# wsntxxn/TextToAudioGrounding

Hardware: AMD Instinct MI355X
Metric: clips/sec (10 s@32 kHz, 1-phrase) fwd+bwd (higher is better)
Workload: dtype f32

## Files before the change

### texttoaudiogrounding_amd/csrc/conv_c1.hip

```cpp
#include "tag_common.h"

namespace {

__device__ __forceinline__ float c1_in(const float* x, const float* cs, const float* ct, int H, int W, long m,
                                       int h, int w, int dy, int dx) {
    const int hh = h + dy, ww = w + dx;
    if (hh < 0 || hh >= H || ww < 0 || ww >= W) return 0.0f;
    const float v = x[m + (long)dy * W + dx];
    return cs ? fmaf(v, cs[ww], ct[ww]) : v;
}

__global__ __launch_bounds__(256) void conv_c1_fwd_kernel(const float* __restrict__ x, const float* __restrict__ cs,
                                                          const float* __restrict__ ct, const float* __restrict__ w,
                                                          float* __restrict__ y, long M, int H, int W, int Cout) {
    const int C4 = Cout >> 2;
    const long total = M * C4;
    for (long i = (long)blockIdx.x * 256 + threadIdx.x; i < total; i += (long)gridDim.x * 256) {
        const int c = (int)(i % C4) << 2;
        const long m = i / C4;
        const int hw = (int)(m % ((long)H * W));
        const int h = hw / W, ww = hw % W;
        float o[4] = {0, 0, 0, 0};
#pragma unroll
        for (int tap = 0; tap < 9; ++tap) {
// ... 194 lines not shown
}

constexpr int C1B_GW = 66, C1B_GT = 10;
__device__ __forceinline__ void c1_stage_row(float (*Xs)[C1B_GW], const float* ximg, const float* cs, const float* ct, int H,
                                             int row) {
    constexpr int W = 64;
    const int tid = threadIdx.x;
    if (tid < C1B_GW) {
        const int w = tid - 1;
        float v = 0.0f;
        if ((unsigned)row < (unsigned)H && (unsigned)w < (unsigned)W) {
            v = ximg[(size_t)row * W + w];
            if (cs) v = fmaf(v, cs[w], ct[w]);
        }
        Xs[(row + 8) & 3][tid] = v;
    }
}

template <class TS>
__global__ __launch_bounds__(256) void conv_c1_fwd_rows_kernel(const float* __restrict__ x, const float* __restrict__ cs,
                                                               const float* __restrict__ ct, const float* __restrict__ wgt,
                                                               TS* __restrict__ y, float* __restrict__ stats, int H,
                                                               int strips, int rows_per_strip) {
    constexpr int W = 64, Cout = 64;
    __shared__ float Xs[4][C1B_GW];
    const int img = blockIdx.x / strips, strip = blockIdx.x % strips;
    const int r0 = strip * rows_per_strip;
    int r1 = r0 + rows_per_strip;
    if (r1 > H) r1 = H;
    const int tid = threadIdx.x, c = (tid & 15) << 2, grp = tid >> 4;
    float wr[4][9];
#pragma unroll
    for (int j = 0; j < 4; ++j)
#pragma unroll
        for (int t = 0; t < 9; ++t) wr[j][t] = wgt[(c + j) * 9 + t];
    const float* ximg = x + (size_t)img * H * W;
    float sk[4] = {0, 0, 0, 0}, sr[4] = {0, 0, 0, 0}, sq[4] = {0, 0, 0, 0};
    bool have_pivot = false;
    c1_stage_row(Xs, ximg, cs, ct, H, r0 - 1);
    c1_stage_row(Xs, ximg, cs, ct, H, r0);
    c1_stage_row(Xs, ximg, cs, ct, H, r0 + 1);
    __syncthreads();
    for (int h = r0; h < r1; ++h) {
        if (h + 2 <= r1) c1_stage_row(Xs, ximg, cs, ct, H, h + 2);
        float xin[3][6];
#pragma unroll
        for (int r = 0; r < 3; ++r)
#pragma unroll
            for (int k = 0; k < 6; ++k) xin[r][k] = Xs[(h + r - 1 + 8) & 3][grp * 4 + k];
        TS* yrow = y + (((size_t)img * H + h) * W + grp * 4) * Cout + c;
#pragma unroll
        for (int px = 0; px < 4; ++px) {
            float o[4] = {0, 0, 0, 0};
#pragma unroll
            for (int tap = 0; tap < 9; ++tap)
#pragma unroll
                for (int j = 0; j < 4; ++j) o[j] = fmaf(xin[tap / 3][px + tap % 3], wr[j][tap], o[j]);
            Act<TS>::st4(yrow + (size_t)px * Cout, (f32x4){o[0], o[1], o[2], o[3]});
            if (stats) {
                if (!have_pivot) {
#pragma unroll
                    for (int j = 0; j < 4; ++j) sk[j] = o[j];
                    have_pivot = true;
                }
#pragma unroll
                for (int j = 0; j < 4; ++j) { const float d = o[j] - sk[j]; sr[j] += d; sq[j] = fmaf(d, d, sq[j]); }
            }
        }
        __syncthreads();
    }
    if (stats) {
        const int P = gridDim.x * 16, prow = blockIdx.x * 16 + grp;
        float* ps = stats + (size_t)prow * 3 * Cout;
#pragma unroll
        for (int j = 0; j < 4; ++j) { ps[c + j] = sk[j]; ps[Cout + c + j] = sr[j]; ps[2 * Cout + c + j] = sq[j]; }
        if (c == 0) stats[(size_t)P * 3 * Cout + prow] = (float)((r1 - r0) * 4);
    }
}

struct C1BnBwd {
    const void* yref; const float* scale; const float* shift; const float* mean; const float* invstd;
    const float* gamma; const float* dgamma; const float* dbeta; float invN; int bn_train;
};
template <class TS, bool FUSE>
__global__ __launch_bounds__(256) void conv_c1_bwd_kernel(const float* __restrict__ x, const float* __restrict__ cs,
                                                          const float* __restrict__ ct, const TS* __restrict__ dy,
                                                          const float* __restrict__ wgt, float* __restrict__ dx,
                                                          double* __restrict__ partials, int H, int strips,
                                                          int rows_per_strip, C1BnBwd bb) {
    constexpr int W = 64, Cout = 64;
    __shared__ float Gs[4][C1B_GW][C1B_GT];
    __shared__ float Xs[4][C1B_GW];
    __shared__ float red[4][16][36];
    const int img = blockIdx.x / strips, strip = blockIdx.x % strips;
    const int r0 = strip * rows_per_strip;
    int r1 = r0 + rows_per_strip;
    if (r1 > H) r1 = H;
    const int tid = threadIdx.x, lane = tid & 63, wid = tid >> 6;
    const int cq = lane & 15, c = cq << 2, psub = lane >> 4;
    const int tapl = lane & 15, kg = lane >> 4;
    const bool tap_ok = tapl < 9;
    const int tky = tap_ok ? tapl / 3 : 0, tkx = tap_ok ? tapl % 3 : 0;
    float wB[16];
#pragma unroll
    for (int q = 0; q < 16; ++q) wB[q] = tap_ok ? wgt[(kg * 16 + q) * 9 + tapl] : 0.0f;
    f32x4 accW[4];
#pragma unroll
    for (int j = 0; j < 4; ++j) accW[j] = (f32x4){0.0f, 0.0f, 0.0f, 0.0f};
    __shared__ __attribute__((aligned(16))) float Ts[4][16][68];
    for (int i = tid; i < 4 * C1B_GW * C1B_GT; i += 256) (&Gs[0][0][0])[i] = 0.0f;
    const float* ximg = x + (size_t)img * H * W;
    const TS* dimg = dy + (size_t)img * H * W * Cout;
    typedef ActN<TS, 4> AN;
    typedef typename AN::raw_t raw_t;
    constexpr int NY = FUSE ? 4 : 1;
    f32x4 g[4];
    raw_t gn[4], yn[NY];
    __shared__ float bnc[7][Cout];
    const TS* yimg = nullptr;
    if constexpr (FUSE) {
        yimg = static_cast<const TS*>(bb.yref) + (size_t)img * H * W * Cout;
        if (tid < Cout) {
            const float is = bb.invstd[tid];
            bnc[0][tid] = bb.scale[tid]; bnc[1][tid] = bb.shift[tid]; bnc[2][tid] = bb.mean[tid]; bnc[3][tid] = is;
            bnc[4][tid] = bb.gamma[tid] * is;
            bnc[5][tid] = bb.bn_train ? bb.dbeta[tid] * bb.invN : 0.0f;
            bnc[6][tid] = bb.bn_train ? bb.dgamma[tid] * bb.invN : 0.0f;
        }
    }
    auto load_dy = [&](int row) {
        const bool ok = (unsigned)row < (unsigned)H;
        const size_t off = ((size_t)(ok ? row : 0) * W + wid * 16 + psub) * Cout + c;
#pragma unroll
        for (int i = 0; i < 4; ++i) {
            gn[i] = AN::ldraw(dimg + off + (size_t)i * 4 * Cout);
            if constexpr (FUSE) yn[i] = AN::ldraw(yimg + off + (size_t)i * 4 * Cout);
            else if (!ok) gn[i] = AN::zero();
        }
    };
    auto take = [&](bool ok) {
        if constexpr (FUSE) {
            float k[7][4];
#pragma unroll
            for (int q = 0; q < 7; ++q) {
                const f32x4 v = *reinterpret_cast<const f32x4*>(&bnc[q][c]);
                k[q][0] = v.x; k[q][1] = v.y; k[q][2] = v.z; k[q][3] = v.w;
            }
#pragma unroll
            for (int i = 0; i < 4; ++i) {
                float av[4], vv[4], o[4];
                AN::unpack(gn[i], av);
                AN::unpack(yn[i], vv);
#pragma unroll
                for (int j = 0; j < 4; ++j) {
                    const float dz = fmaf(vv[j], k[0][j], k[1][j]) > 0.0f ? av[j] : 0.0f;
                    o[j] = k[4][j] * (dz - k[5][j] - (vv[j] - k[2][j]) * k[3][j] * k[6][j]);
                    if (!ok) o[j] = 0.0f;
                }
                g[i] = (f32x4){o[0], o[1], o[2], o[3]};
            }
        } else {
#pragma unroll
            for (int i = 0; i < 4; ++i) {
                float av[4];
                AN::unpack(gn[i], av);
                g[i] = (f32x4){av[0], av[1], av[2], av[3]};
            }
        }
    };
    c1_stage_row(Xs, ximg, cs, ct, H, r0 - 1);
    c1_stage_row(Xs, ximg, cs, ct, H, r0);
    load_dy(r0 - 1);
    __syncthreads();
    take((unsigned)(r0 - 1) < (unsigned)H);
    for (int h = r0 - 1; h <= r1; ++h) {
        c1_stage_row(Xs, ximg, cs, ct, H, h + 2 > r1 + 1 ? -1 : h + 2);
        if (h < r1) load_dy(h + 1);
        const bool own = h >= r0 && h < r1;
        const int gs = (h + 8) & 3;
        if (own) {
#pragma unroll
            for (int i = 0; i < 4; ++i) {
                const float xb = tap_ok ? Xs[(h + tky - 1 + 8) & 3][wid * 16 + i * 4 + psub + tkx] : 0.0f;
                accW[0] = __builtin_amdgcn_mfma_f32_16x16x4f32(g[i].x, xb, accW[0], 0, 0, 0);
                accW[1] = __builtin_amdgcn_mfma_f32_16x16x4f32(g[i].y, xb, accW[1], 0, 0, 0);
                accW[2] = __builtin_amdgcn_mfma_f32_16x16x4f32(g[i].z, xb, accW[2], 0, 0, 0);
                accW[3] = __builtin_amdgcn_mfma_f32_16x16x4f32(g[i].w, xb, accW[3], 0, 0, 0);
            }
        }
#pragma unroll
        for (int i = 0; i < 4; ++i) *reinterpret_cast<f32x4*>(&Ts[wid][i * 4 + psub][c]) = g[i];
        __builtin_amdgcn_fence(__ATOMIC_RELEASE, "wavefront");
        __builtin_amdgcn_wave_barrier();
        __builtin_amdgcn_fence(__ATOMIC_ACQUIRE, "wavefront");
        f32x4 accG = (f32x4){0.0f, 0.0f, 0.0f, 0.0f};
#pragma unroll
        for (int q4 = 0; q4 < 4; ++q4) {
            const f32x4 v = *reinterpret_cast<const f32x4*>(&Ts[wid][tapl][kg * 16 + 4 * q4]);
            accG = __builtin_amdgcn_mfma_f32_16x16x4f32(v.x, wB[4 * q4 + 0], accG, 0, 0, 0);
            accG = __builtin_amdgcn_mfma_f32_16x16x4f32(v.y, wB[4 * q4 + 1], accG, 0, 0, 0);
            accG = __builtin_amdgcn_mfma_f32_16x16x4f32(v.z, wB[4 * q4 + 2], accG, 0, 0, 0);
            accG = __builtin_amdgcn_mfma_f32_16x16x4f32(v.w, wB[4 * q4 + 3], accG, 0, 0, 0);
        }
        if (tap_ok) {
            float* gp = &Gs[gs][wid * 16 + 4 * kg + 1][tapl];
            gp[0] = accG.x; gp[C1B_GT] = accG.y; gp[2 * C1B_GT] = accG.z; gp[3 * C1B_GT] = accG.w;
        }
        __syncthreads();
        const int ho = h - 1;
        if (ho >= r0 && ho < r1 && tid < W) {
            float sdx = 0.0f;
#pragma unroll
            for (int t = 0; t < 9; ++t)
                sdx += Gs[(ho - (t / 3 - 1) + 8) & 3][tid + 1 - (t % 3 - 1)][t];
            dx[((size_t)img * H + ho) * W + tid] = sdx;
        }
        if (h < r1) take((unsigned)(h + 1) < (unsigned)H);
    }
    if (tap_ok) {
#pragma unroll
        for (int j = 0; j < 4; ++j) {
            red[wid][4 * kg + 0][j * 9 + tapl] = accW[j].x;
            red[wid][4 * kg + 1][j * 9 + tapl] = accW[j].y;
            red[wid][4 * kg + 2][j * 9 + tapl] = accW[j].z;
            red[wid][4 * kg + 3][j * 9 + tapl] = accW[j].w;
        }
    }
    __syncthreads();
    for (int e = tid; e < 16 * 36; e += 256) {
        const int q = e / 36, r = e % 36;
        const double sum = ((double)red[0][q][r] + (double)red[1][q][r]) + ((double)red[2][q][r] + (double)red[3][q][r]);
        partials[(size_t)blockIdx.x * Cout * 9 + (q * 4 + r / 9) * 9 + r % 9] = sum;
    }
}

}

static void c1_bwd_geom(int B, int H, int* strips, int* rows) {
    int s = 2048 / (B > 0 ? B : 1);
    if (s < 1) s = 1;
    int r = (H + s - 1) / s;
    if (r < 8) r = 8;
    *rows = r;
    *strips = (H + r - 1) / r;
}
static int c1_blocks(long items, long per_block) {
    const long nb = (items + per_block - 1) / per_block;
    return (int)(nb > 8192 ? 8192 : nb);
}
template <class TS>
static int c1_fwd_rows_launch(const float* x, const float* col_scale, const float* col_shift, const float* w, TS* y,
                              float* stats, int B, int H, void* stream) {
    int strips, rows;
    c1_bwd_geom(B, H, &strips, &rows);
    hipLaunchKernelGGL(conv_c1_fwd_rows_kernel<TS>, dim3(B * strips), dim3(256), 0, as_stream(stream), x, col_scale, col_shift, w,
                       y, stats, H, strips, rows);
    TAG_LAUNCH_CHECK();
    return 0;
}

extern "C" int tag_conv3x3_c1_forward(const float* x, const float* col_scale, const float* col_shift, const float* w,
                                      float* y, int B, int H, int W, int Cout, void* stream) {
    TAG_CHECK_ARG(x && w && y && B > 0 && H > 0 && W > 0 && Cout > 0);
    TAG_CHECK_ARG(Cout % 4 == 0 && (col_scale == nullptr) == (col_shift == nullptr));
    const long M = (long)B * H * W;
    if (W == 64 && Cout == 64) return c1_fwd_rows_launch<float>(x, col_scale, col_shift, w, y, nullptr, B, H, stream);
    if (W % 4 == 0 && 256 % (Cout / 4) == 0)
        hipLaunchKernelGGL(conv_c1_fwd4_kernel<false>, dim3(c1_blocks((M / 4) * (Cout / 4), 256)), dim3(256), 0,
                           as_stream(stream), x, col_scale, col_shift, w, (const float*)nullptr, y, M, H, W, Cout);
    else
        hipLaunchKernelGGL(conv_c1_fwd_kernel, dim3(c1_blocks(M * (Cout / 4), 256)), dim3(256), 0, as_stream(stream), x,
                           col_scale, col_shift, w, y, M, H, W, Cout);
    TAG_LAUNCH_CHECK();
    return 0;
}

extern "C" int tag_conv3x3_c1_forward_bias(const float* x, const float* col_scale, const float* col_shift, const float* w,
                                           const float* bias, float* y, int B, int H, int W, int Cout, void* stream) {
    TAG_CHECK_ARG(x && w && bias && y && B > 0 && H > 0 && (col_scale == nullptr) == (col_shift == nullptr));
    if (!(W > 0 && W % 4 == 0 && Cout >= 4 && Cout % 4 == 0 && 256 % (Cout / 4) == 0)) {
        tag_set_error("%s", "tag_conv3x3_c1_forward_bias: unserved shape (W a multiple of 4, Cout / 4 a divisor of 256)");
        return TAG_EINVAL;
    }
    const long M = (long)B * H * W;
    hipLaunchKernelGGL(conv_c1_fwd4_kernel<true>, dim3(c1_blocks((M / 4) * (Cout / 4), 256)), dim3(256), 0, as_stream(stream), x,
                       col_scale, col_shift, w, bias, y, M, H, W, Cout);
    TAG_LAUNCH_CHECK();
    return 0;
}

extern "C" int tag_conv3x3_c1_stats_rows(int B, int H, int W, int Cout) {
    if (!(W == 64 && Cout == 64 && B > 0 && H > 0)) return 0;
    int strips, rows;
    c1_bwd_geom(B, H, &strips, &rows);
    return B * strips * 16;
}
extern "C" int tag_conv3x3_c1_forward_stats(const float* x, const float* col_scale, const float* col_shift, const float* w,
                                            float* y, float* stats, int B, int H, int W, int Cout, void* stream) {
    TAG_CHECK_ARG(x && w && y && stats && W == 64 && Cout == 64 && B > 0 && H > 0);
    TAG_CHECK_ARG((col_scale == nullptr) == (col_shift == nullptr));
    return c1_fwd_rows_launch<float>(x, col_scale, col_shift, w, y, stats, B, H, stream);
}
extern "C" int tag_conv3x3_c1_forward_stats_bf16(const float* x, const float* col_scale, const float* col_shift,
                                                 const float* w, void* y, float* stats, int B, int H, int W, int Cout,
                                                 void* stream) {
    TAG_CHECK_ARG(x && w && y && W == 64 && Cout == 64 && B > 0 && H > 0);
    TAG_CHECK_ARG((col_scale == nullptr) == (col_shift == nullptr));
    return c1_fwd_rows_launch<bf16_t>(x, col_scale, col_shift, w, static_cast<bf16_t*>(y), stats, B, H, stream);
}

extern "C" size_t tag_conv3x3_c1_wgrad_ws_bytes(int B, int H, int W, int Cout) {
    (void)B; (void)H; (void)W;
    return (size_t)1024 * Cout * 9 * sizeof(double);
}

extern "C" int tag_conv3x3_c1_wgrad(const float* x, const float* col_scale, const float* col_shift, const float* dy,
                                    float* dw, int B, int H, int W, int Cout, void* ws, void* stream) {
    TAG_CHECK_ARG(x && dy && dw && ws && B > 0 && H > 0 && W > 0 && Cout > 0);
    TAG_CHECK_ARG(Cout % 4 == 0 && Cout / 4 <= 64 && 64 % (Cout / 4) == 0);
    TAG_CHECK_ARG((col_scale == nullptr) == (col_shift == nullptr));
    const long M = (long)B * H * W;
    const int rpi = 256 / (Cout / 4);
    long nb = (M + (long)rpi * 64 - 1) / ((long)rpi * 64);
    const int nblk = (int)(nb > 1024 ? 1024 : (nb < 1 ? 1 : nb));
    double* partials = static_cast<double*>(ws);
    hipLaunchKernelGGL(W % 4 == 0 ? conv_c1_wgrad_kernel<4> : conv_c1_wgrad_kernel<1>, dim3(nblk), dim3(256),
                       4 * 64 * 36 * sizeof(double), as_stream(stream), x, col_scale, col_shift, dy, partials, M, H, W, Cout);
    TAG_LAUNCH_CHECK();
    hipLaunchKernelGGL(conv_c1_wgrad_finalize_kernel, dim3(cdiv(Cout * 9, 8)), dim3(256), 0, as_stream(stream),
                       partials, nblk, Cout * 9, dw);
    TAG_LAUNCH_CHECK();
    return 0;
}

extern "C" int tag_conv3x3_c1_dgrad(const float* dy, const float* w, float* dx, int B, int H, int W, int Cout,
                                    void* stream) {
    TAG_CHECK_ARG(dy && w && dx && B > 0 && H > 0 && W > 0 && Cout > 0);
    TAG_CHECK_ARG(Cout % 4 == 0 && Cout / 4 <= 64 && 64 % (Cout / 4) == 0);
    const long M = (long)B * H * W;
    const int rpi = 256 / (Cout / 4);
    hipLaunchKernelGGL(conv_c1_dgrad_kernel, dim3(c1_blocks(M, rpi)), dim3(256), 0, as_stream(stream), dy, w, dx, M, H, W, Cout);
    TAG_LAUNCH_CHECK();
    return 0;
}

extern "C" size_t tag_conv3x3_c1_backward_ws_bytes(int B, int H, int W, int Cout) {
    (void)W;
    int strips, rows;
    c1_bwd_geom(B, H, &strips, &rows);
    return (size_t)B * strips * Cout * 9 * sizeof(double);
}
template <class TS>
static int c1_backward_impl(const float* x, const float* col_scale, const float* col_shift, const TS* dy, const float* w,
                            float* dw, float* dx, int B, int H, int W, int Cout, void* ws, void* stream, const C1BnBwd* bb) {
    TAG_CHECK_ARG(x && dy && w && dw && dx && ws && B > 0 && H > 0);
    TAG_CHECK_ARG(W == 64 && Cout == 64);
    TAG_CHECK_ARG((col_scale == nullptr) == (col_shift == nullptr));
    int strips, rows;
    c1_bwd_geom(B, H, &strips, &rows);
    double* partials = static_cast<double*>(ws);
    if (bb) {
        TAG_CHECK_ARG(bb->yref && bb->scale && bb->shift && bb->mean && bb->invstd && bb->gamma && bb->dgamma && bb->dbeta);
        hipLaunchKernelGGL((conv_c1_bwd_kernel<TS, true>), dim3(B * strips), dim3(256), 0, as_stream(stream), x, col_scale,
                           col_shift, dy, w, dx, partials, H, strips, rows, *bb);
    } else {
        hipLaunchKernelGGL((conv_c1_bwd_kernel<TS, false>), dim3(B * strips), dim3(256), 0, as_stream(stream), x, col_scale,
                           col_shift, dy, w, dx, partials, H, strips, rows, C1BnBwd{});
    }
    TAG_LAUNCH_CHECK();
    hipLaunchKernelGGL(conv_c1_wgrad_finalize_kernel, dim3(cdiv(Cout * 9, 8)), dim3(256), 0, as_stream(stream),
                       partials, B * strips, Cout * 9, dw);
    TAG_LAUNCH_CHECK();
    return 0;
}
extern "C" int tag_conv3x3_c1_backward(const float* x, const float* col_scale, const float* col_shift, const float* dy,
                                       const float* w, float* dw, float* dx, int B, int H, int W, int Cout, void* ws,
                                       void* stream) {
    return c1_backward_impl<float>(x, col_scale, col_shift, dy, w, dw, dx, B, H, W, Cout, ws, stream, nullptr);
}
extern "C" int tag_conv3x3_c1_backward_bf16(const float* x, const float* col_scale, const float* col_shift, const void* dy,
                                            const float* w, float* dw, float* dx, int B, int H, int W, int Cout, void* ws,
                                            void* stream) {
    return c1_backward_impl<bf16_t>(x, col_scale, col_shift, static_cast<const bf16_t*>(dy), w, dw, dx, B, H, W, Cout, ws,
                                    stream, nullptr);
}
static C1BnBwd c1_bn_bwd(const void* yref, const float* bn_scale, const float* bn_shift, const float* bn_mean,
                         const float* bn_invstd, const float* gamma, const float* dgamma, const float* dbeta, int bn_train,
                         int B, int H, int W) {
    return C1BnBwd{yref, bn_scale, bn_shift, bn_mean, bn_invstd, gamma, dgamma, dbeta, 1.0f / (float)((long)B * H * W), bn_train};
}
extern "C" int tag_conv3x3_c1_backward_bnrelu(const float* x, const float* col_scale, const float* col_shift, const float* da,
                                              const float* yref, const float* bn_scale, const float* bn_shift,
                                              const float* bn_mean, const float* bn_invstd, const float* gamma,
                                              const float* dgamma, const float* dbeta, int bn_train, const float* w,
                                              float* dw, float* dx, int B, int H, int W, int Cout, void* ws, void* stream) {
    const C1BnBwd bb = c1_bn_bwd(yref, bn_scale, bn_shift, bn_mean, bn_invstd, gamma, dgamma, dbeta, bn_train, B, H, W);
    return c1_backward_impl<float>(x, col_scale, col_shift, da, w, dw, dx, B, H, W, Cout, ws, stream, &bb);
}
extern "C" int tag_conv3x3_c1_backward_bnrelu_bf16(const float* x, const float* col_scale, const float* col_shift,
                                                   const void* da, const void* yref, const float* bn_scale,
                                                   const float* bn_shift, const float* bn_mean, const float* bn_invstd,
                                                   const float* gamma, const float* dgamma, const float* dbeta, int bn_train,
                                                   const float* w, float* dw, float* dx, int B, int H, int W, int Cout,
                                                   void* ws, void* stream) {
    const C1BnBwd bb = c1_bn_bwd(yref, bn_scale, bn_shift, bn_mean, bn_invstd, gamma, dgamma, dbeta, bn_train, B, H, W);
    return c1_backward_impl<bf16_t>(x, col_scale, col_shift, static_cast<const bf16_t*>(da), w, dw, dx, B, H, W, Cout, ws,
                                    stream, &bb);
}
```

### texttoaudiogrounding_amd/csrc/tag_lib.hip

```cpp
#include <stdarg.h>
#include <string.h>
#include "tag_common.h"

static thread_local char g_err[512] = "";

void tag_set_error(const char* fmt, ...) {
    va_list ap;
    va_start(ap, fmt);
    vsnprintf(g_err, sizeof(g_err), fmt, ap);
    va_end(ap);
}

#ifndef TAG_CSRC_SHA256
#define TAG_CSRC_SHA256 "unknown"
#endif
namespace {
struct TagOpt { const char* name; int value; };
TagOpt g_opts[] = {
    {"conv_impl", 0},
    {"halo_lds_pad", 0},
    {"halo_bn256", 1},
    {"wgrad_wgs", 512},
    {"conv_rows", 1},
    {"wgrad_dma", 1},
    {"x3_products", 6},
    {"gemm_big_min", 2048},
    {"gru_tile4", 1},
    {"gru_xcd", 1},
    {"gru_coop", 1},
    {"mha_mfma", 1},
};
}
int tag_option(const char* name) {
    for (const TagOpt& o : g_opts)
        if (strcmp(o.name, name) == 0) return o.value;
    return 0;
}
extern "C" int tag_set_option(const char* name, int value) {
    TAG_CHECK_ARG(name != nullptr);
    for (TagOpt& o : g_opts)
        if (strcmp(o.name, name) == 0) { o.value = value; return 0; }
    tag_set_error("tag_set_option: unknown option '%s'", name);
    return TAG_EINVAL;
}

extern "C" int tag_abi_version(void) { return TAG_ABI_VERSION; }
extern "C" const char* tag_build_id(void) { return TAG_CSRC_SHA256; }
extern "C" const char* tag_last_error(void) { return g_err; }
extern "C" int tag_device_cu_count(void) {
    int dev = 0, n = 0;
    if (hipGetDevice(&dev) != hipSuccess) return -1;
    if (hipDeviceGetAttribute(&n, hipDeviceAttributeMultiprocessorCount, dev) != hipSuccess) return -1;
    return n;
}

extern "C" int tag_stream_create_cu_mask(const unsigned* mask, int words, void** stream_out) {
    TAG_CHECK_ARG(mask && words > 0 && stream_out);
    hipStream_t st = nullptr;
    const hipError_t e = hipExtStreamCreateWithCUMask(&st, (uint32_t)words, mask);
    if (e != hipSuccess) {
        tag_set_error("hipExtStreamCreateWithCUMask failed: %s", hipGetErrorString(e));
        (void)hipGetLastError();
        return (int)e;
    }
    *stream_out = reinterpret_cast<void*>(st);
    return 0;
}
```

### texttoaudiogrounding_amd/dispatch.py

```python
from __future__ import annotations

import collections
import math
from typing import Optional

import torch

from . import settings as cfg
from .lib import call, ptr, query
from .engine import (F32, _chk, _empty, _timed, _ws)


def waveform_f16_to_f32_padded(clips, device, length=None):
    import numpy as np
    arrs = [c.numpy() if isinstance(c, torch.Tensor) else np.asarray(c) for c in clips]
    if any(a.dtype != np.float16 or a.ndim != 1 for a in arrs):
        raise RuntimeError("waveform_f16_to_f32_padded: clips must be 1-D float16 arrays (the pack's storage type)")
    lens = [a.shape[0] for a in arrs]
    S = int(length) if length is not None else max(lens)
    off = torch.tensor([0] + list(np.cumsum(lens)), dtype=torch.long)
    packed = torch.from_numpy(np.concatenate(arrs) if len(arrs) > 1 else arrs[0].copy())
    dev = torch.device(device)
    if dev.type != "cuda":
        raise RuntimeError("waveform_f16_to_f32_padded: the target must be the MI355X (cuda) device; no CPU fallback")
# ... 318 lines not shown
            ws = _ws(query("tag_conv3x3_wino_ws_bytes", b1 - b0, H, W, Cin, Cout), x)
            with _timed(("conv3x3_wino", b1 - b0, H, W, Cin, Cout), _wino_flop(b1 - b0, H, W, Cin, Cout)):
                call("tag_conv3x3_wino_forward_bnrelu_pool_eval", ptr(x[b0:b1]), ptr(u), prologue, ptr(scale), ptr(shift),
                     ptr(out[b0:b1]), ptr(st.scale), ptr(st.shift), b1 - b0, H, W, Cin, Cout, ph, pw, int(pool), ptr(ws))
        return out
    with _timed(("conv3x3_halo_kernel", B, H, W, Cin, Cout), 2.0 * B * H * W * 9 * Cin * Cout):
        call("tag_conv3x3_forward_bnrelu_pool_eval", ptr(x), ptr(wpack), prologue, ptr(scale), ptr(shift), ptr(out), ptr(st.scale),
             ptr(st.shift), B, H, W, Cin, Cout, ph, pw, int(pool))
    return out


def conv3x3_wgrad(x, dy, prologue=0, scale=None, shift=None, out=None):
    B, H, W, Cin = x.shape
    Cout = dy.shape[3]
    dw = out if out is not None else _empty(Cout, Cin, 3, 3, like=x)
    if x.dtype == BF16:
        if dy.dtype != BF16 or not (W in (8, 16, 32, 64) and Cin % 64 == 0 and Cout % 64 == 0):
            raise RuntimeError("bf16 wgrad: both operands must be bf16, width 8/16/32/64, channels multiples of 64")
        ws = _ws(query("tag_conv3x3_wgrad_x3_ws_bytes", B, H, W, Cin, Cout), x)
        with _timed(("conv3x3_wgrad_x3_kernel", B, H, W, Cin, Cout), 2.0 * B * H * W * 9 * Cin * Cout):
            call("tag_conv3x3_wgrad_x3_bf16", ptr(x), prologue, ptr(scale), ptr(shift), ptr(dy), ptr(dw), B, H, W, Cin, Cout,
                 ptr(ws))
        return dw
    if cfg.CONV_MATH in _X3_PRODUCTS and W in (8, 16, 32, 64) and Cin % 64 == 0 and Cout % 64 == 0:
        ws = _ws(query("tag_conv3x3_wgrad_x3_ws_bytes", B, H, W, Cin, Cout), x)
        with _timed(("conv3x3_wgrad_x3_kernel", B, H, W, Cin, Cout), 2.0 * B * H * W * 9 * Cin * Cout):
            call("tag_conv3x3_wgrad_x3", ptr(x), prologue, ptr(scale), ptr(shift), ptr(dy), ptr(dw), B, H, W, Cin, Cout,
                 _X3_PRODUCTS[cfg.CONV_MATH], ptr(ws))
        return dw
    if (x.dtype == F32 and dy.dtype == F32 and _wino_shape(W, Cin, Cout)
            and B * ((H + 1) // 2) * ((W + 1) // 2) * max(Cin, Cout) >= cfg.WINO_MIN_WORK and query("tag_conv3x3_wino_ok", B, H, W, Cin, Cout)):
        cfg.WINO_LAUNCHES += 1
        ws = _ws(query("tag_conv3x3_wino_wgrad_ws_bytes", B, H, W, Cin, Cout), x)
        with _timed(("conv3x3_wino_wgrad", B, H, W, Cin, Cout), _wino_flop(B, H, W, Cin, Cout)):
            call("tag_conv3x3_wino_wgrad", ptr(x), prologue, ptr(scale), ptr(shift), ptr(dy), ptr(dw), B, H, W, Cin, Cout, ptr(ws),
                 None)
        return dw
    ws = _ws(query("tag_conv3x3_wgrad_ws_bytes", B, H, W, Cin, Cout), x)
    kname = "conv3x3_wgrad_alltaps_kernel" if W in (8, 16, 32, 64) else "conv3x3_wgrad_kernel"
    with _timed((kname, B, H, W, Cin, Cout), 2.0 * B * H * W * 9 * Cin * Cout):
        call("tag_conv3x3_wgrad", ptr(x), prologue, ptr(scale), ptr(shift), ptr(dy), ptr(dw), B, H, W, Cin, Cout,
             ptr(ws))
    return dw


def conv3x3_c1(x, w, col_scale=None, col_shift=None):
    return conv3x3_c1_stats(x, w, col_scale, col_shift, want_stats=False)[0]


def conv3x3_c1_stats(x, w, col_scale=None, col_shift=None, want_stats=True, out_dtype=F32):
    B, H, W = x.shape
    Cout = w.shape[0]
    y = _empty(B, H, W, Cout, like=x, dtype=out_dtype)
    if out_dtype == BF16:
        P = query("tag_conv3x3_c1_stats_rows", B, H, W, Cout)
        if P <= 0:
            raise RuntimeError("bf16 activations: the Cin = 1 convolution is implemented for 64 mel bins x 64 channels")
        part = (P, _empty(P * (3 * Cout + 1), like=x)) if want_stats else None
        call("tag_conv3x3_c1_forward_stats_bf16", ptr(x), ptr(col_scale), ptr(col_shift), ptr(w), ptr(y),
             ptr(part[1]) if part else None, B, H, W, Cout)
        return y, part
    P = query("tag_conv3x3_c1_stats_rows", B, H, W, Cout) if (want_stats and cfg.FUSE_BN_STATS) else 0
    if P > 0:
        part = (P, _empty(P * (3 * Cout + 1), like=x))
        call("tag_conv3x3_c1_forward_stats", ptr(x), ptr(col_scale), ptr(col_shift), ptr(w), ptr(y), ptr(part[1]), B, H, W,
             Cout)
        return y, part
    call("tag_conv3x3_c1_forward", ptr(x), ptr(col_scale), ptr(col_shift), ptr(w), ptr(y), B, H, W, Cout)
    return y, None


def conv3x3_c1_wgrad(x, dy, col_scale=None, col_shift=None, out=None):
    B, H, W = x.shape
    Cout = dy.shape[3]
    dw = out if out is not None else _empty(Cout, 1, 3, 3, like=x)
    ws = _ws(query("tag_conv3x3_c1_wgrad_ws_bytes", B, H, W, Cout), x)
    call("tag_conv3x3_c1_wgrad", ptr(x), ptr(col_scale), ptr(col_shift), ptr(dy), ptr(dw), B, H, W, Cout, ptr(ws))
    return dw


C1_BWD_FUSED_SHAPE = (64, 64)


def conv3x3_c1_backward(x, dy, w, col_scale=None, col_shift=None, out=None, bn_bwd=None):
    B, H, W = x.shape
    Cout = dy.shape[3]
    if (W, Cout) == C1_BWD_FUSED_SHAPE:
        dw = out if out is not None else _empty(Cout, 1, 3, 3, like=x)
        dx = _empty(B, H, W, like=x)
        ws = _ws(query("tag_conv3x3_c1_backward_ws_bytes", B, H, W, Cout), x)
        if bn_bwd is not None:
            yref, st, gamma, dg, db = bn_bwd
            if yref.dtype != dy.dtype or yref.shape != dy.shape:
                raise RuntimeError("conv3x3_c1_backward: yref and da must agree in dtype and shape")
            call("tag_conv3x3_c1_backward_bnrelu" + _sfx(dy), ptr(x), ptr(col_scale), ptr(col_shift), ptr(dy), ptr(yref),
                 ptr(st.scale), ptr(st.shift), ptr(st.mean), ptr(st.invstd), ptr(gamma), ptr(dg), ptr(db), int(st.train),
                 ptr(w), ptr(dw), ptr(dx), B, H, W, Cout, ptr(ws))
            return dw, dx
        call("tag_conv3x3_c1_backward" + _sfx(dy), ptr(x), ptr(col_scale), ptr(col_shift), ptr(dy), ptr(w), ptr(dw), ptr(dx),
             B, H, W, Cout, ptr(ws))
        return dw, dx
    if bn_bwd is not None:
        raise RuntimeError("conv3x3_c1_backward: bn_bwd needs the fused 64 x 64 shape")
    if dy.dtype == BF16:
        raise RuntimeError("bf16 activations: the Cin = 1 backward is implemented for 64 mel bins x 64 channels")
    return conv3x3_c1_wgrad(x, dy, col_scale, col_shift), conv3x3_c1_dgrad(dy, w)


def conv3x3_c1_dgrad(dy, w):
    B, H, W, Cout = dy.shape
    dx = _empty(B, H, W, like=dy)
    call("tag_conv3x3_c1_dgrad", ptr(dy), ptr(w), ptr(dx), B, H, W, Cout)
    return dx


def bnact_pool(y, st: Optional[BNStat], ph, pw, act=1, pool=0, drop_p=0.0, seed=0):
    B, H, W, C = y.shape
    out = _empty(B, H // ph, W // pw, C, like=y, dtype=y.dtype)
    call("tag_bnact_pool_forward" + _sfx(y), ptr(y), ptr(st.scale) if st else None, ptr(st.shift) if st else None, ptr(out), B,
         H, W, C, ph, pw, act, pool, float(drop_p), seed)
    return out


def bnrelu_pool_backward(y, st: BNStat, gamma, dout, ph, pw, drop_p=0.0, seed=0, dg_out=None, db_out=None, pool=0,
                         partials=None):
    B, H, W, C = y.shape
    if dout.dtype != y.dtype:
        raise RuntimeError("bnrelu_pool_backward: y and dout must share their storage type")
    dy = _empty(B, H, W, C, like=y, dtype=y.dtype)
    dg, db = _dg_db(dg_out, db_out, C, y)
    if partials is not None:
        P, part = partials
        ws = _ws(query("tag_bn_grad_from_partials_ws_bytes", P, C), y)
        call("tag_bn_grad_from_partials", ptr(part), P, C, ptr(dg), ptr(db), ptr(ws))
        call("tag_bnrelu_pool_backward_apply" + _sfx(y), ptr(y), ptr(st.scale), ptr(st.shift), ptr(st.mean), ptr(st.invstd),
             ptr(gamma), ptr(dout), ptr(dy), ptr(dg), ptr(db), B, H, W, C, ph, pw, int(pool), float(drop_p), seed, int(st.train))
        return dy, dg, db
    ws = _ws(query("tag_bn_backward_ws_bytes", B * H * W, C), y)
    call("tag_bnrelu_pool_backward" + _sfx(y), ptr(y), ptr(st.scale), ptr(st.shift), ptr(st.mean), ptr(st.invstd), ptr(gamma),
         ptr(dout), ptr(dy), ptr(dg), ptr(db), B, H, W, C, ph, pw, int(pool), float(drop_p), seed, int(st.train), ptr(ws))
    return dy, dg, db


def bnrelu_backward(y, st: BNStat, gamma, da, inplace=True, dg_out=None, db_out=None):
    C = y.shape[-1]
    rows = y.numel() // C
    dy = da if inplace else torch.empty_like(da)
    dg, db = _dg_db(dg_out, db_out, C, y)
    ws = _ws(query("tag_bn_backward_ws_bytes", rows, C), y)
    if da.dtype != y.dtype:
        raise RuntimeError("bnrelu_backward: y and da must share their storage type")
    call("tag_bnrelu_backward" + _sfx(y), ptr(y), ptr(st.scale), ptr(st.shift), ptr(st.mean), ptr(st.invstd), ptr(gamma),
         ptr(da), ptr(dy), ptr(dg), ptr(db), rows, C, int(st.train), ptr(ws))
    return dy, dg, db


def bn_param_grad(x2d, dy2d, st: BNStat, dg_out=None, db_out=None):
    rows, C = x2d.shape
    dg, db = _dg_db(dg_out, db_out, C, x2d)
    ws = _ws(query("tag_bn_backward_ws_bytes", rows, C), x2d)
    call("tag_bn_param_grad", ptr(x2d), ptr(dy2d), rows, C, ptr(st.mean), ptr(st.invstd), ptr(dg), ptr(db), ptr(ws))
    return dg, db


def _stripe_counts(stripes, n_time, B):
    if stripes is None:
        return 0, 0
    if (not stripes.is_cuda or not stripes.is_contiguous() or stripes.dtype != torch.int32 or stripes.dim() != 3
            or stripes.shape[0] != B or stripes.shape[2] != 2):
        raise RuntimeError(f"augment: stripes must be a contiguous device int32 (B={B}, n_time + n_freq, 2) table, got "
                           f"{stripes.dtype} {tuple(stripes.shape)} on {stripes.device}")
    if not 0 <= n_time <= stripes.shape[1]:
        raise RuntimeError(f"augment: n_time {n_time} outside the table's {stripes.shape[1]} rows")
    return n_time, stripes.shape[1] - n_time


def augment_forward(lm, scale=None, shift=None, stripes=None, n_time=0, lam=None):
    lm = _chk(lm, "lm")
    B, Fr, NM = lm.shape
    nt, nf = _stripe_counts(stripes, n_time, B)
# ... 1988 lines not shown
```

### texttoaudiogrounding_amd/functions.py

```python
from __future__ import annotations

from typing import List, Optional

import torch

from . import settings as cfg
from .lib import call, ptr, query
from .engine import (F32, TagFunction, _chk, _deliver, _empty, _flush, _ready, _side_stream, _sinks, _ws, new_seed,
                     side_stream_enabled)
from .dispatch import (BF16, BNStat, C1_BWD_FUSED_SHAPE, _sfx, _wino_u, act_bf16, augment_backward, augment_forward,
                       bn_act_backward, bn_param_grad,
                       bn_stats, bnact_pool, bnrelu_pool_backward, check_pass_size, colsum, conv3x3,
                       conv3x3_bnrelu_pool_eval, conv3x3_c1, conv3x3_c1_backward, conv3x3_c1_dgrad, conv3x3_c1_stats,
                       conv3x3_c1_wgrad, conv3x3_dgrad_bnrelu_backward, conv3x3_dgrad_poolsums, conv3x3_stats,
                       conv3x3_wgrad, embed_mean_backward_into, embed_mean_forward, eval_pool_fusable, gemm,
                       gru_bidir_backward, gru_bidir_forward, logmel, lppool_leaky_backward, pack_conv_weight,
                       pool_sums_fusable, relu_backward)
from .dispatch import (bias_bnrelu_backward, bias_bnrelu_forward, bias_bnrelu_pool, bias_bnrelu_pool_backward,
                       bn_act_backward_clip, conv3x3_bias, conv3x3_c1_bias, frame_head_backward, frame_head_forward, gemm_bf16, leaky_backward,
                       leaky_forward, lppool_leaky_backward_clip, rowgroup_bias_relu, rowgroup_colsum)
from .dispatch import class_pool_forward, tagging_head_dlogit
from .dispatch import text_gru_backward, text_gru_forward
from .dispatch import text_selfattn_backward, text_selfattn_forward
from .dispatch import text_clap_backward, text_clap_forward
# ... 21 lines not shown
        if not cfg.WGRAD_LAG:
            self.release()
        return dw

    def run(self, fn, tensors=()):
        if not self.on:
            fn()
            return
        self.release()
        self.side.wait_stream(self.main)
        with torch.cuda.stream(self.side):
            fn()
        self._hold(tensors)

    def release(self):
        if not self.pending:
            return
        self.side.wait_stream(self.main)
        with torch.cuda.stream(self.side):
            for x, dy, prologue, scale, shift, dw in self.pending:
                conv3x3_wgrad(x, dy, prologue, scale, shift, out=dw)
        for item in self.pending:
            self._hold(item)
        self.pending = []

    def _hold(self, tensors):
        for t in tensors:
            if isinstance(t, torch.Tensor):
                if cfg.SIDE_RECORD_STREAM:
                    t.record_stream(self.side)
                else:
                    self.keep.append(t)

    def join(self):
        if self.on:
            self.release()
            self.main.wait_stream(self.side)
            self.keep = []


def _cnn8_begin(waveform, mod, params):
    wave = _chk(waveform, "waveform")
    check_pass_size(wave.shape[0], wave.shape[1] // mod.hop_length + 1)
    training = mod.training
    p = [_chk(t.detach(), "parameter") for t in params]
    drop = mod.dropout_p if training else (0.0, 0.0)
    seeds = [new_seed() for _ in range(5)] if training and (drop[0] > 0 or drop[1] > 0) else [0] * 5
    return wave, p, training and not mod.freeze_bn, drop, seeds


def _cnn8_stem_forward(wave, mod, p, bn_train, aug, out_dtype=F32):
    lm = logmel(wave, mod.n_fft, mod.win_length, mod.hop_length, mod.window, mod.mel_fb)
    B, Fr, NM = lm.shape
    st0 = bn_stats(lm.view(B * Fr, NM), p[0], p[1], mod.bn0.running_mean, mod.bn0.running_var, bn_train, mod.bn0.eps,
                   mod.bn0.momentum)
    if aug is None:
        x0 = None
        y1, part1 = conv3x3_c1_stats(lm, p[2], st0.scale, st0.shift, want_stats=bn_train, out_dtype=out_dtype)
    else:
        x0 = augment_forward(lm, st0.scale, st0.shift, *aug)
        y1, part1 = conv3x3_c1_stats(x0, p[2], None, None, want_stats=bn_train, out_dtype=out_dtype)
    return lm, st0, x0, y1, part1


def _cnn8_tail_forward(x, fc_w, fc_b, drop_p, seed, act):
    Bx, Tp, Wp, C = x.shape
    xm = _empty(Bx * Tp, C, like=x)
    call("tag_mean_w_forward" + _sfx(x), ptr(x), Bx * Tp, Wp, C, float(drop_p), seed, ptr(xm))
    return xm, gemm(xm, fc_w, Bx * Tp, fc_w.shape[0], C, transB=True, bias=fc_b, act=act)


def _cnn8_tail_backward(dfc, fc_w, x_last, drop_p, seed):
    M = dfc.shape[0]
    dxm = gemm(dfc, fc_w, M, fc_w.shape[1], fc_w.shape[0])
    Bx, Tp, Wp, C = x_last.shape
    dx = torch.empty_like(x_last)
    call("tag_mean_w_backward" + _sfx(dx), ptr(dxm), Bx * Tp, Wp, C, float(drop_p), seed, ptr(dx))
    return dx


def _cnn8_stem_backward(sv, dy1, grads, sk, bn_bwd=None):
    lm, st0, x0 = sv["lm"], sv["st0"], sv["x0"]
    if x0 is None:
        dw0, dbn0 = conv3x3_c1_backward(lm, dy1, sv["p"][2], st0.scale, st0.shift, out=sk[2], bn_bwd=bn_bwd)
    else:
        dw0, dx0 = conv3x3_c1_backward(x0, dy1, sv["p"][2], None, None, out=sk[2], bn_bwd=bn_bwd)
        dbn0 = augment_backward(dx0, lm.shape[0], *sv["aug"])
        del dx0
    _deliver(grads, sk, 2, dw0)
    Bq, Fr, NM = lm.shape
    dg0, db0 = bn_param_grad(lm.view(Bq * Fr, NM), dbn0.view(Bq * Fr, NM), st0, dg_out=sk[0], db_out=sk[1])
    _deliver(grads, sk, 0, dg0)
    _deliver(grads, sk, 1, db0)


def _cnn8_block_done(sw, prm, i):
    sw.release()
    if prm is not None:
        o = 2 + 6 * i
        _ready(prm[o:o + 6] + ((prm[0], prm[1]) if i == 0 else ()))
        _flush()


class Cnn8RnnFunction(TagFunction):

    @staticmethod
    def forward(ctx, waveform, mod, *params):
        wave, p, bn_train, drop, seeds = _cnn8_begin(waveform, mod, params)
        need_grad = any(ctx.needs_input_grad[2:])
        aug = getattr(ctx, "augment", None)
        lm, st0, x0, y1, part1 = _cnn8_stem_forward(wave, mod, p, bn_train, aug, out_dtype=BF16 if act_bf16() else F32)
        x = wd1 = None
        acts = []
        for i in range(4):
            c1w, g1, b1, c2w, g2, b2 = p[2 + 6 * i: 8 + 6 * i]
            blk = getattr(mod, f"conv_block{i + 1}")
            if i > 0:
                wf1, wd1 = pack_conv_weight(c1w, want_dgrad=need_grad, W=x.shape[2])
                y1, part1 = conv3x3_stats(x, wf1, c1w.shape[0], want_stats=bn_train,
                                          inference=not need_grad and not bn_train and drop[0] == 0.0)
            Bx, H, W, C = y1.shape
            s1 = bn_stats(y1.view(-1, C), g1, b1, blk.bn1.running_mean, blk.bn1.running_var, bn_train, blk.bn1.eps,
                          blk.bn1.momentum, partials=part1)
            wf2, wd2 = pack_conv_weight(c2w, want_dgrad=need_grad, W=y1.shape[2])
            ph, pw = CNN8_POOLS[i]
            if not need_grad and not bn_train and drop[0] == 0.0 and eval_pool_fusable(y1, wf2, ph, pw):
                s2 = bn_stats(g2.view(1, C), g2, b2, blk.bn2.running_mean, blk.bn2.running_var, False, blk.bn2.eps, blk.bn2.momentum)
                x = conv3x3_bnrelu_pool_eval(y1, wf2, C, s2, ph, pw, prologue=1, scale=s1.scale, shift=s1.shift)
                continue
            y2, part2 = conv3x3_stats(y1, wf2, C, prologue=1, scale=s1.scale, shift=s1.shift, want_stats=bn_train)
            s2 = bn_stats(y2.view(-1, C), g2, b2, blk.bn2.running_mean, blk.bn2.running_var, bn_train, blk.bn2.eps,
                          blk.bn2.momentum, partials=part2)
            xo = bnact_pool(y2, s2, ph, pw, act=1, pool=0, drop_p=drop[0], seed=seeds[i])
            if need_grad:
                acts.append((x, y1, s1, y2, s2, wd1, wd2))
            x = xo
        xm, fc = _cnn8_tail_forward(x, p[26], p[27], drop[1], seeds[4], act=1)
        y, gsave = gru_bidir_forward(fc, p[28:36], x.shape[0], x.shape[1], need_grad)
        if need_grad:
            ctx.saved = dict(lm=lm, st0=st0, aug=aug, x0=x0, acts=acts, x_last=x, xm=xm, fc=fc, gsave=gsave, p=p, drop=drop,
                             seeds=seeds, sinks=_sinks(params), params=params if cfg.DIRECT_GRADS else None)
        mod._last_dropout = dict(p=drop, seeds=seeds)
        return y

    @staticmethod
    def backward(ctx, dy):
        sv = ctx.saved
        ctx.saved = None
        p = sv["p"]
        drop, seeds = sv["drop"], sv["seeds"]
        dy = _chk(dy, "grad_output")
        grads: List[Optional[torch.Tensor]] = [None] * len(p)
        sk, prm = sv["sinks"], sv["params"]
        fc = sv["fc"]
        sw = _SideWgrad(dy.device)
        dfc, ggru = gru_bidir_backward(dy, fc, sv["gsave"], outs=sk[28:36], side=sw if cfg.SIDE_PARAM_GRADS >= 1 else None)
        for k in range(8):
            _deliver(grads, sk, 28 + k, ggru[k])
        M = fc.shape[0]
        dfc = relu_backward(fc, dfc)
        xm = sv["xm"]
        fc_w = p[26]
        if cfg.SIDE_PARAM_GRADS >= 2 and sk[26] is not None and sk[27] is not None:
            sw.run(lambda: (gemm(dfc, xm, fc_w.shape[0], fc_w.shape[1], M, transA=True, lda=fc_w.shape[0], out=sk[26]),
                            colsum(dfc, M, fc_w.shape[0], out=sk[27])), (dfc, xm))
            _deliver(grads, sk, 26, sk[26])
            _deliver(grads, sk, 27, sk[27])
        else:
            _deliver(grads, sk, 26, gemm(dfc, xm, fc_w.shape[0], fc_w.shape[1], M, transA=True, lda=fc_w.shape[0], out=sk[26]))
# ... 1167 lines not shown
```

Measured before the change: 2037.

## Recompute stem conv output in fused c1 backward instead of reloading y1

Adds a template variant of the Cin=1 conv backward kernel that recomputes the 3x3 conv output y1 from the staged input rows and shared-memory weights, instead of reading the stored y1 tensor for the fused BN+ReLU backward. This removes a full 64-channel activation read from HBM and replaces it with 36 FMAs per output group, which is cheap for a single input channel. The stem backward enables the variant through a temporary global option toggle. The kernel also gains a launch_bounds occupancy hint of 3 blocks per CU, and one extra input row is staged for the recompute halo.

Result: no change. 2043 (median of 6 runs) (+0.3%).

```diff
diff --git a/texttoaudiogrounding_amd/csrc/conv_c1.hip b/texttoaudiogrounding_amd/csrc/conv_c1.hip
--- a/texttoaudiogrounding_amd/csrc/conv_c1.hip
+++ b/texttoaudiogrounding_amd/csrc/conv_c1.hip
@@ -300,8 +300,8 @@
     const void* yref; const float* scale; const float* shift; const float* mean; const float* invstd;
     const float* gamma; const float* dgamma; const float* dbeta; float invN; int bn_train;
 };
-template <class TS, bool FUSE>
-__global__ __launch_bounds__(256) void conv_c1_bwd_kernel(const float* __restrict__ x, const float* __restrict__ cs,
+template <class TS, bool FUSE, bool RC = false>
+__global__ __launch_bounds__(256, 3) void conv_c1_bwd_kernel(const float* __restrict__ x, const float* __restrict__ cs,
                                                           const float* __restrict__ ct, const TS* __restrict__ dy,
                                                           const float* __restrict__ wgt, float* __restrict__ dx,
                                                           double* __restrict__ partials, int H, int strips,
@@ -331,13 +331,19 @@
     const TS* dimg = dy + (size_t)img * H * W * Cout;
     typedef ActN<TS, 4> AN;
     typedef typename AN::raw_t raw_t;
-    constexpr int NY = FUSE ? 4 : 1;
+    static_assert((FUSE && !Act<TS>::is_bf16) || !RC, "the recomputed y1 only feeds the fused BatchNorm backward of fp32 storage");
+    constexpr int NY = FUSE && !RC ? 4 : 1;
     f32x4 g[4];
     raw_t gn[4], yn[NY];
     __shared__ float bnc[7][Cout];
+    __shared__ __attribute__((aligned(16))) float Wt[RC ? 9 : 1][Cout];
     const TS* yimg = nullptr;
     if constexpr (FUSE) {
-        yimg = static_cast<const TS*>(bb.yref) + (size_t)img * H * W * Cout;
+        if constexpr (RC) {
+            for (int e = tid; e < 9 * Cout; e += 256) Wt[e % 9][e / 9] = wgt[e];
+        } else {
+            yimg = static_cast<const TS*>(bb.yref) + (size_t)img * H * W * Cout;
+        }
         if (tid < Cout) {
             const float is = bb.invstd[tid];
             bnc[0][tid] = bb.scale[tid]; bnc[1][tid] = bb.shift[tid]; bnc[2][tid] = bb.mean[tid]; bnc[3][tid] = is;
@@ -352,12 +358,21 @@
 #pragma unroll
         for (int i = 0; i < 4; ++i) {
             gn[i] = AN::ldraw(dimg + off + (size_t)i * 4 * Cout);
-            if constexpr (FUSE) yn[i] = AN::ldraw(yimg + off + (size_t)i * 4 * Cout);
-            else if (!ok) gn[i] = AN::zero();
+            if constexpr (FUSE && !RC) yn[i] = AN::ldraw(yimg + off + (size_t)i * 4 * Cout);
+            else if constexpr (!FUSE) { if (!ok) gn[i] = AN::zero(); }
         }
     };
-    auto take = [&](bool ok) {
+    auto take = [&](int row) {
+        const bool ok = (unsigned)row < (unsigned)H;
         if constexpr (FUSE) {
+            float wv[RC ? 9 : 1][4];
+            if constexpr (RC) {
+#pragma unroll
+                for (int t = 0; t < 9; ++t) {
+                    const f32x4 v = *reinterpret_cast<const f32x4*>(&Wt[t][c]);
+                    wv[t][0] = v.x; wv[t][1] = v.y; wv[t][2] = v.z; wv[t][3] = v.w;
+                }
+            }
             float k[7][4];
 #pragma unroll
             for (int q = 0; q < 7; ++q) {
@@ -368,7 +383,19 @@
             for (int i = 0; i < 4; ++i) {
                 float av[4], vv[4], o[4];
                 AN::unpack(gn[i], av);
-                AN::unpack(yn[i], vv);
+                if constexpr (RC) {
+                    float xv[9];
+#pragma unroll
+                    for (int t = 0; t < 9; ++t) xv[t] = Xs[(row + t / 3 - 1 + 8) & 3][wid * 16 + i * 4 + psub + t % 3];
+#pragma unroll
+                    for (int j = 0; j < 4; ++j) vv[j] = 0.0f;
+#pragma unroll
+                    for (int t = 0; t < 9; ++t)
+#pragma unroll
+                        for (int j = 0; j < 4; ++j) vv[j] = fmaf(xv[t], wv[t][j], vv[j]);
+                } else {
+                    AN::unpack(yn[i], vv);
+                }
 #pragma unroll
                 for (int j = 0; j < 4; ++j) {
                     const float dz = fmaf(vv[j], k[0][j], k[1][j]) > 0.0f ? av[j] : 0.0f;
@@ -386,13 +413,14 @@
             }
         }
     };
+    if constexpr (RC) c1_stage_row(Xs, ximg, cs, ct, H, r0 - 2);
     c1_stage_row(Xs, ximg, cs, ct, H, r0 - 1);
     c1_stage_row(Xs, ximg, cs, ct, H, r0);
     load_dy(r0 - 1);
     __syncthreads();
-    take((unsigned)(r0 - 1) < (unsigned)H);
+    take(r0 - 1);
     for (int h = r0 - 1; h <= r1; ++h) {
-        c1_stage_row(Xs, ximg, cs, ct, H, h + 2 > r1 + 1 ? -1 : h + 2);
+        if (h + 2 <= r1 + 1) c1_stage_row(Xs, ximg, cs, ct, H, h + 2);
         if (h < r1) load_dy(h + 1);
         const bool own = h >= r0 && h < r1;
         const int gs = (h + 8) & 3;
@@ -433,7 +461,7 @@
                 sdx += Gs[(ho - (t / 3 - 1) + 8) & 3][tid + 1 - (t % 3 - 1)][t];
             dx[((size_t)img * H + ho) * W + tid] = sdx;
         }
-        if (h < r1) take((unsigned)(h + 1) < (unsigned)H);
+        if (h < r1) take(h + 1);
     }
     if (tap_ok) {
 #pragma unroll
@@ -579,8 +607,13 @@
     double* partials = static_cast<double*>(ws);
     if (bb) {
         TAG_CHECK_ARG(bb->yref && bb->scale && bb->shift && bb->mean && bb->invstd && bb->gamma && bb->dgamma && bb->dbeta);
-        hipLaunchKernelGGL((conv_c1_bwd_kernel<TS, true>), dim3(B * strips), dim3(256), 0, as_stream(stream), x, col_scale,
-                           col_shift, dy, w, dx, partials, H, strips, rows, *bb);
+        constexpr bool can_recompute = !Act<TS>::is_bf16;
+        if (can_recompute && tag_option("c1_bwd_recompute"))
+            hipLaunchKernelGGL((conv_c1_bwd_kernel<TS, true, can_recompute>), dim3(B * strips), dim3(256), 0, as_stream(stream), x,
+                               col_scale, col_shift, dy, w, dx, partials, H, strips, rows, *bb);
+        else
+            hipLaunchKernelGGL((conv_c1_bwd_kernel<TS, true>), dim3(B * strips), dim3(256), 0, as_stream(stream), x, col_scale,
+                               col_shift, dy, w, dx, partials, H, strips, rows, *bb);
     } else {
         hipLaunchKernelGGL((conv_c1_bwd_kernel<TS, false>), dim3(B * strips), dim3(256), 0, as_stream(stream), x, col_scale,
                            col_shift, dy, w, dx, partials, H, strips, rows, C1BnBwd{});
diff --git a/texttoaudiogrounding_amd/csrc/tag_lib.hip b/texttoaudiogrounding_amd/csrc/tag_lib.hip
--- a/texttoaudiogrounding_amd/csrc/tag_lib.hip
+++ b/texttoaudiogrounding_amd/csrc/tag_lib.hip
@@ -29,6 +29,7 @@
     {"gru_xcd", 1},
     {"gru_coop", 1},
     {"mha_mfma", 1},
+    {"c1_bwd_recompute", 0},
 };
 }
 int tag_option(const char* name) {
diff --git a/texttoaudiogrounding_amd/dispatch.py b/texttoaudiogrounding_amd/dispatch.py
--- a/texttoaudiogrounding_amd/dispatch.py
+++ b/texttoaudiogrounding_amd/dispatch.py
@@ -424,7 +424,7 @@
 C1_BWD_FUSED_SHAPE = (64, 64)
 
 
-def conv3x3_c1_backward(x, dy, w, col_scale=None, col_shift=None, out=None, bn_bwd=None):
+def conv3x3_c1_backward(x, dy, w, col_scale=None, col_shift=None, out=None, bn_bwd=None, yref_is_y1=False):
     B, H, W = x.shape
     Cout = dy.shape[3]
     if (W, Cout) == C1_BWD_FUSED_SHAPE:
@@ -435,9 +435,15 @@
             yref, st, gamma, dg, db = bn_bwd
             if yref.dtype != dy.dtype or yref.shape != dy.shape:
                 raise RuntimeError("conv3x3_c1_backward: yref and da must agree in dtype and shape")
-            call("tag_conv3x3_c1_backward_bnrelu" + _sfx(dy), ptr(x), ptr(col_scale), ptr(col_shift), ptr(dy), ptr(yref),
-                 ptr(st.scale), ptr(st.shift), ptr(st.mean), ptr(st.invstd), ptr(gamma), ptr(dg), ptr(db), int(st.train),
-                 ptr(w), ptr(dw), ptr(dx), B, H, W, Cout, ptr(ws))
+            if yref_is_y1:
+                query("tag_set_option", b"c1_bwd_recompute", 1)
+            try:
+                call("tag_conv3x3_c1_backward_bnrelu" + _sfx(dy), ptr(x), ptr(col_scale), ptr(col_shift), ptr(dy), ptr(yref),
+                     ptr(st.scale), ptr(st.shift), ptr(st.mean), ptr(st.invstd), ptr(gamma), ptr(dg), ptr(db), int(st.train),
+                     ptr(w), ptr(dw), ptr(dx), B, H, W, Cout, ptr(ws))
+            finally:
+                if yref_is_y1:
+                    query("tag_set_option", b"c1_bwd_recompute", 0)
             return dw, dx
         call("tag_conv3x3_c1_backward" + _sfx(dy), ptr(x), ptr(col_scale), ptr(col_shift), ptr(dy), ptr(w), ptr(dw), ptr(dx),
              B, H, W, Cout, ptr(ws))
diff --git a/texttoaudiogrounding_amd/functions.py b/texttoaudiogrounding_amd/functions.py
--- a/texttoaudiogrounding_amd/functions.py
+++ b/texttoaudiogrounding_amd/functions.py
@@ -127,9 +127,9 @@
 def _cnn8_stem_backward(sv, dy1, grads, sk, bn_bwd=None):
     lm, st0, x0 = sv["lm"], sv["st0"], sv["x0"]
     if x0 is None:
-        dw0, dbn0 = conv3x3_c1_backward(lm, dy1, sv["p"][2], st0.scale, st0.shift, out=sk[2], bn_bwd=bn_bwd)
+        dw0, dbn0 = conv3x3_c1_backward(lm, dy1, sv["p"][2], st0.scale, st0.shift, out=sk[2], bn_bwd=bn_bwd, yref_is_y1=True)
     else:
-        dw0, dx0 = conv3x3_c1_backward(x0, dy1, sv["p"][2], None, None, out=sk[2], bn_bwd=bn_bwd)
+        dw0, dx0 = conv3x3_c1_backward(x0, dy1, sv["p"][2], None, None, out=sk[2], bn_bwd=bn_bwd, yref_is_y1=True)
         dbn0 = augment_backward(dx0, lm.shape[0], *sv["aug"])
         del dx0
     _deliver(grads, sk, 2, dw0)
```
